# CrystalSixone/VLN-GOAT

Hardware: AMD Instinct MI355X
Metric: trajectory-steps/sec fwd+bwd (GOAT pretrain, 36 views x 768, 80 tok) (higher is better)
Workload: dtype bf16

## Files before the change

include/goat_hip.h:

```cpp
#ifndef GOAT_HIP_H
#define GOAT_HIP_H

#include <stdint.h>

#ifdef __cplusplus
extern "C" {
#endif

#define GOAT_F32 0
#define GOAT_BF16 1

#define GOAT_E_ARG (-1)
#define GOAT_E_SHAPE (-2)

#define GOAT_EPI_NONE 0
#define GOAT_EPI_GELU 1
#define GOAT_EPI_RELU 2
#define GOAT_EPI_MUL_DGELU 3
#define GOAT_EPI_MUL_DRELU 4
#define GOAT_EPI_ACCUM 5

int goat_version(void);

int goat_gemm_nt(void* stream, int dtype_in, int dtype_out,
                 const void* A, int64_t lda, const void* B, int64_t ldb, void* C, int64_t ldc,
                 int M, int N, int K, const float* bias, int epilogue,
                 void* aux, int64_t ldaux, int split_k);

#define GOAT_GEMM_8WAVES 0x100
#define GOAT_GEMM_PP 0x200
#define GOAT_GEMM_PERSIST 0x400

int goat_gemm_bf16(void* stream, int trans_a, int trans_b, int dtype_out,
                   const void* A, int64_t lda, const void* B, int64_t ldb, void* C, int64_t ldc,
                   int M, int N, int Kc, const float* bias, int epilogue,
                   void* aux, int64_t ldaux, int split_k, int bm, int nstage, float* colsum);
int goat_colsum(void* stream, int dtype, const void* x, int64_t ld, int R, int C, float* colsum);

int goat_wgrad_smallk(void* stream, int dtype, const void* dy, int64_t ld_dy, const void* x, int64_t ld_x, int rows, int N, int K,
                      float* dw, int64_t ld_dw, float* dbias);

int goat_transpose(void* stream, int dtype, const void* in, int64_t ld_in, void* out, int64_t ld_out,
                   int R, int C, float* colsum);

int goat_ln_fwd(void* stream, int dtype, const void* x, const void* residual,
                const float* gamma, const float* beta, float eps,
                float p, uint64_t seed, uint64_t offset, const uint64_t* rng_dev,
                void* y, void* z_out, float* mean, float* rstd, int M, int H);

#define GOAT_LN_ADD_BEFORE 4
typedef struct goat_ln_partial {
  const float* ws;
  float* dgamma;
  float* dbeta;
  int32_t nparts;
  int32_t reserved;
} goat_ln_partial;
int goat_ln_bwd_ws_floats(int H);
int goat_ln_bwd_nparts(int M);
// ... 177 lines not shown
```

vln-goat_amd/_lib.py:

```python
import ctypes
import glob
import os
import subprocess

import torch

_HERE = os.path.dirname(os.path.abspath(__file__))
CSRC = os.path.join(_HERE, 'csrc')
LIB_PATH = os.environ.get('GOAT_HIP_LIB') or os.path.join(CSRC, 'libgoat_hip.so')
SOURCES = ['gemm.hip', 'gemm2.hip', 'gemm3.hip', 'gemm5.hip', 'attention.hip', 'attention2.hip', 'attention_long.hip', 'decode.hip', 'rowops.hip', 'causal.hip', 'optim.hip', 'glue.hip']

GOAT_F32, GOAT_BF16 = 0, 1
EPI_NONE, EPI_GELU, EPI_RELU, EPI_MUL_DGELU, EPI_MUL_DRELU, EPI_ACCUM = 0, 1, 2, 3, 4, 5

_lib = None

_vp = ctypes.c_void_p
_i32 = ctypes.c_int
_i64 = ctypes.c_int64
_u64 = ctypes.c_uint64
_f32 = ctypes.c_float

SIGNATURES = {
    'goat_version': [],
    'goat_gemm_nt': [_vp, _i32, _i32, _vp, _i64, _vp, _i64, _vp, _i64, _i32, _i32, _i32, _vp, _i32, _vp, _i64, _i32],
    'goat_gemm_bf16': [_vp, _i32, _i32, _i32, _vp, _i64, _vp, _i64, _vp, _i64, _i32, _i32, _i32, _vp, _i32, _vp, _i64, _i32, _i32, _i32, _vp],
    'goat_colsum': [_vp, _i32, _vp, _i64, _i32, _i32, _vp],
    'goat_transpose': [_vp, _i32, _vp, _i64, _vp, _i64, _i32, _i32, _vp],
    'goat_ln_fwd': [_vp, _i32, _vp, _vp, _vp, _vp, _f32, _f32, _u64, _u64, _vp, _vp, _vp, _vp, _vp, _i32, _i32],
    'goat_wgrad_smallk': [_vp, _i32, _vp, _i64, _vp, _i64, _i32, _i32, _i32, _vp, _i64, _vp],
    'goat_ln_bwd_ws_floats': [_i32],
    'goat_ln_bwd_nparts': [_i32],
    'goat_ln_reduce_batched': [_vp, _vp, _i32, _i32],
    'goat_ln_bwd': [_vp, _i32, _vp, _vp, _vp, _vp, _vp, _vp, _f32, _u64, _u64, _vp, _vp, _vp, _vp, _vp, _vp, _i32, _i32, _i32, _vp],
    'goat_ln_fwd_do': [_vp, _i32, _vp, _vp, _vp, _vp, _f32, _f32, _u64, _u64, _vp, _vp, _vp, _vp, _vp, _i32, _i32, _f32, _u64, _vp],
    'goat_ln_bwd_do': [_vp, _i32, _vp, _vp, _vp, _vp, _vp, _vp, _f32, _u64, _u64, _vp, _vp, _vp, _vp, _vp, _vp, _i32, _i32, _i32, _vp, _f32, _u64, _vp],
    'goat_dropout_add_fwd': [_vp, _i32, _vp, _vp, _vp, _i64, _f32, _u64, _u64, _vp],
    'goat_dropout_bwd': [_vp, _i32, _vp, _vp, _i64, _f32, _u64, _u64, _vp],
    'goat_act_bwd': [_vp, _i32, _vp, _vp, _vp, _i64, _i32, _f32, _u64, _u64, _vp],
    'goat_attn_fwd': [_vp, _i32] + [_vp, _i64, _i64] * 4 + [_vp, _vp, _vp, _i32, _i32, _i32, _i32, _f32, _f32, _u64, _u64, _vp],
    'goat_attn_bwd': [_vp, _i32] + [_vp, _i64, _i64] * 8 + [_vp, _vp, _vp, _vp, _i32, _i32, _i32, _i32, _f32, _f32, _u64, _u64, _vp],
    'goat_attn_long_fwd': [_vp, _i32] + [_vp, _i64, _i64] * 4 + [_vp, _vp, _vp, _i32, _i32, _i32, _i32, _f32, _f32, _u64, _u64, _vp],
    'goat_attn_long_bwd': [_vp, _i32] + [_vp, _i64, _i64] * 8 + [_vp, _vp, _vp, _vp, _i32, _i32, _i32, _i32, _f32, _f32, _u64, _u64, _vp],
    'goat_attn_decode_fwd': [_vp, _i32, _vp, _vp, _vp, _i64, _i64, _vp, _vp, _vp, _i32, _i32, _i32, _f32, _f32, _u64, _u64, _vp],
    'goat_decode_select': [_vp, _vp, _i64, _i32, _i32, _i32, _i32, _i32, _i32, _i32, _u64, _u64, _vp, _vp, _vp, _vp, _vp, _vp, _vp],
    'goat_ce_fwd': [_vp, _vp, _i64, _i32, _i32, _vp, _vp, _vp],
    'goat_ce_bwd': [_vp, _i32, _vp, _i64, _i32, _i32, _vp, _vp, _vp, _vp, _i64],
    'goat_pano_fusion_fwd': [_vp, _i32, _vp, _vp, _vp, _vp, _vp, _i32, _i32, _i32],
    'goat_pano_fusion_bwd': [_vp, _i32, _vp, _vp, _vp, _vp, _vp, _vp, _vp, _vp, _i32, _i32, _i32],
# ... 98 lines not shown
```

vln-goat_amd/csrc/gemm2.hip:

```cpp
#include "gemm5_tile.hpp"

using namespace goat_g2;

static int pick_group_m(int tiles_m, int tiles_n, int bm, int bn) {
  if (const char* e = getenv("GOAT_GEMM_GROUP_M")) {
    int g = atoi(e);
    return g < 1 ? 1 : (g > tiles_m ? tiles_m : g);
  }
  static std::mutex mu;
  static std::unordered_map<uint64_t, int> cache;
  const uint64_t key = ((uint64_t)tiles_m << 44) | ((uint64_t)tiles_n << 24) | ((uint64_t)bm << 12) | (uint64_t)bn;
  {
    std::lock_guard<std::mutex> lk(mu);
    auto it = cache.find(key);
    if (it != cache.end()) return it->second;
  }
  const int nwg = tiles_m * tiles_n, q = nwg >> 3, r = nwg & 7;
  int best = 1;
  double best_cost = 1e300;
  std::vector<char> seen_m(tiles_m), seen_n(tiles_n);
  const int gmax = tiles_m < 64 ? tiles_m : 64;
  for (int gm = 1; gm <= gmax; ++gm) {
    double cost = 0;
    int pos = 0;
// ... 10 lines not shown
        if (!seen_n[tn]) { seen_n[tn] = 1; ++dn; }
      }
      cost += (double)dm * bm + (double)dn * bn;
    }
    if (cost < best_cost - 1e-9) { best_cost = cost; best = gm; }
  }
  std::lock_guard<std::mutex> lk(mu);
  cache[key] = best;
  return best;
}


static bool tile_ok(int bm, int bn, bool eight) {
  if (bn == 128 && bm == 96) return !eight;
  if (bn == 128) return bm == 64 || bm == 128 || bm == 256 ? (!eight || bm == 128) : false;
  if (eight) return false;
  return (bm == 128 && bn == 256) || (bm == 192 && bn == 256) || (bm == 256 && bn == 192) || (bm == 256 && bn == 256) || (bm == 192 && bn == 192);
}

static bool pp_tile_ok(int bm, int bn, int nstage) {
  return nstage == 2 && ((bm == 256 && bn == 256) || (bm == 192 && bn == 256) || (bm == 128 && bn == 256) || (bm == 256 && bn == 128) || (bm == 128 && bn == 128));
}

extern "C" int goat_gemm_bf16(void* stream, int trans_a, int trans_b, int dtype_out,
                              const void* A, int64_t lda, const void* B, int64_t ldb, void* C, int64_t ldc,
                              int M, int N, int Kc, const float* bias, int epilogue,
                              void* aux, int64_t ldaux, int split_k, int bm, int nstage, float* colsum) {
  if (!A || !B || !C) return GOAT_E_ARG;
  const bool eight = (nstage & GOAT_GEMM_8WAVES) != 0;
  const bool pp = (nstage & GOAT_GEMM_PP) != 0;
  const bool persist = (nstage & GOAT_GEMM_PERSIST) != 0;
  nstage &= ~(GOAT_GEMM_8WAVES | GOAT_GEMM_PP | GOAT_GEMM_PERSIST);
  if (nstage < 2 || nstage > 4) return GOAT_E_ARG;
  if (persist && !pp) return GOAT_E_ARG;
  int bn = (bm >> 16) & 0xFFFF;
  bm &= 0xFFFF;
  if (bn == 0) bn = 128;
  if (colsum && !trans_a) return GOAT_E_ARG;
  if (M <= 0 || N <= 0 || Kc <= 0) return GOAT_E_SHAPE;
  if ((lda % 8) || (ldb % 8)) return GOAT_E_SHAPE;
  if ((reinterpret_cast<uintptr_t>(A) & 15) || (reinterpret_cast<uintptr_t>(B) & 15)) return GOAT_E_SHAPE;
  if ((!trans_a || !trans_b) && (Kc % BK)) return GOAT_E_SHAPE;
  if (trans_a && !trans_b) return GOAT_E_ARG;
  if ((epilogue == GOAT_EPI_MUL_DGELU || epilogue == GOAT_EPI_MUL_DRELU) && (!aux || bias)) return GOAT_E_ARG;
  if (epilogue == GOAT_EPI_ACCUM && (dtype_out != GOAT_F32 || bias)) return GOAT_E_ARG;
  if (split_k > 1 && (dtype_out != GOAT_F32 || (epilogue != GOAT_EPI_NONE && epilogue != GOAT_EPI_ACCUM) || bias)) return GOAT_E_ARG;
  if (pp ? (eight || !pp_tile_ok(bm, bn, nstage)) : !tile_ok(bm, bn, eight)) return GOAT_E_ARG;
  const int64_t a_rows = trans_a ? Kc : M, b_rows = trans_b ? Kc : N;
  const int64_t a_bytes = a_rows * lda * 2, b_bytes = b_rows * ldb * 2;
  if (a_bytes >= (1ll << 31) || b_bytes >= (1ll << 31)) return GOAT_E_SHAPE;

  G2Args a;
  a.A = A; a.B = B; a.C = C; a.bias = bias; a.aux = aux;
  a.lda = lda; a.ldb = ldb; a.ldc = ldc; a.ldaux = ldaux;
  a.M = M; a.N = N; a.Kc = Kc;
  a.tiles_m = (M + bm - 1) / bm;
  a.tiles_n = (N + bn - 1) / bn;
  a.a_bytes = (uint32_t)a_bytes; a.b_bytes = (uint32_t)b_bytes;
  a.colsum = colsum;
  a.accum = epilogue == GOAT_EPI_ACCUM;
  a.group_m = pick_group_m(a.tiles_m, a.tiles_n, bm, bn);
  const int kt = (Kc + BK - 1) / BK;
  if (split_k < 1) split_k = 1;
  if (split_k > kt) split_k = kt;
  a.k_tiles_per_split = (kt + split_k - 1) / split_k;
  hipStream_t st = reinterpret_cast<hipStream_t>(stream);
  if (pp) return goat_g5_dispatch(st, a, bm, bn, trans_a, trans_b, dtype_out, epilogue, split_k, nstage, persist);
  if (bn != 128 || bm == 96) return goat_g3_dispatch(st, a, bm, bn, trans_a, trans_b, dtype_out, epilogue, split_k, nstage);
  if (bm == 64) return dispatch_layout<T64>(st, a, trans_a, trans_b, dtype_out, epilogue, split_k, nstage);
  if (bm == 256) return dispatch_layout<T256>(st, a, trans_a, trans_b, dtype_out, epilogue, split_k, nstage);
  if (eight) return dispatch_layout<T128X8>(st, a, trans_a, trans_b, dtype_out, epilogue, split_k, nstage);
  return dispatch_layout<T128>(st, a, trans_a, trans_b, dtype_out, epilogue, split_k, nstage);
}

template <class CF>
static int group_stages(hipStream_t st, const GroupArgs& g, int nstage) {
  constexpr int STAGE = smem_bytes<CF, true, true, 1>();
  if (nstage == 2) return launch_group<CF, 2>(st, g);
  if constexpr (3 * STAGE <= 160 * 1024) {
    if (nstage == 3) return launch_group<CF, 3>(st, g);
  }
  if constexpr (4 * STAGE <= 160 * 1024 && CF::BM * CF::BN <= 128 * 128) {
    if (nstage == 4) return launch_group<CF, 4>(st, g);
  }
  return GOAT_E_ARG;
}

static int build_group(const goat_wgrad_problem* probs, int n, int bm, int bn, GroupArgs& g) {
  g.n = n;
  int tiles = 0;
  for (int i = 0; i < n; ++i) {
    const goat_wgrad_problem& q = probs[i];
    if (!q.dy || !q.x || !q.dw) return GOAT_E_ARG;
    if (q.rows <= 0 || q.n_out <= 0 || q.n_in <= 0) return GOAT_E_SHAPE;
    if ((q.ld_dy % 8) || (q.ld_x % 8)) return GOAT_E_SHAPE;
// ... 58 lines not shown
```

vln-goat_amd/csrc/gemm2_tile.hpp:

```cpp
#pragma once
#include <algorithm>
#include <cstdlib>
#include <mutex>
#include <type_traits>
#include <unordered_map>
#include <vector>
#include "gemm_epilogue.hpp"

namespace goat_g2 {

constexpr int BK = 64;
#ifndef GOAT_GEMM_FRAG_DEPTH
#define GOAT_GEMM_FRAG_DEPTH 2
#endif
#ifndef GOAT_G2_ROTATED
#define GOAT_G2_ROTATED 0
#endif
#ifndef GOAT_G2_SPREAD
#define GOAT_G2_SPREAD 1
#endif
#ifndef GOAT_G2_SETPRIO
#define GOAT_G2_SETPRIO 0
#endif
#ifndef GOAT_G2_NOEPI
// ... 464 lines not shown
template <class F>
int with_epilogue(int epi, F&& f) {
  switch (epi) {
    case GOAT_EPI_NONE: return f(std::integral_constant<int, GOAT_EPI_NONE>());
    case GOAT_EPI_GELU: return f(std::integral_constant<int, GOAT_EPI_GELU>());
    case GOAT_EPI_RELU: return f(std::integral_constant<int, GOAT_EPI_RELU>());
    case GOAT_EPI_MUL_DGELU: return f(std::integral_constant<int, GOAT_EPI_MUL_DGELU>());
    case GOAT_EPI_MUL_DRELU: return f(std::integral_constant<int, GOAT_EPI_MUL_DRELU>());
  }
  return GOAT_E_ARG;
}

template <class CF, bool TA, bool TB>
int dispatch2(hipStream_t st, const G2Args& a, int dtype_out, int epi, int split, int nstage) {
  if (split > 1) return launch2<CF, TA, TB, float, GOAT_EPI_NONE, true>(st, a, split, nstage);
  if (dtype_out == GOAT_F32) {
    if (epi != GOAT_EPI_NONE && epi != GOAT_EPI_ACCUM) return GOAT_E_ARG;
    return launch2<CF, TA, TB, float, GOAT_EPI_NONE, false>(st, a, 1, nstage);
  }
  if constexpr (TA) {
    if (epi != GOAT_EPI_NONE) return GOAT_E_ARG;
    return launch2<CF, TA, TB, bf16_t, GOAT_EPI_NONE, false>(st, a, 1, nstage);
  }
  return with_epilogue(epi, [&](auto e) { return launch2<CF, TA, TB, bf16_t, decltype(e)::value, false>(st, a, 1, nstage); });
}

template <class CF>
int dispatch_layout(hipStream_t st, const G2Args& a, int trans_a, int trans_b, int dtype_out, int epi, int split, int nstage) {
  constexpr bool POW2_M = (CF::BM & (CF::BM - 1)) == 0, POW2_N = (CF::BN & (CF::BN - 1)) == 0;
  if (!trans_a && !trans_b) return dispatch2<CF, false, false>(st, a, dtype_out, epi, split, nstage);
  if constexpr (POW2_N) {
    if (!trans_a && trans_b) return dispatch2<CF, false, true>(st, a, dtype_out, epi, split, nstage);
    if constexpr (POW2_M) {
      if (trans_a && trans_b) return dispatch2<CF, true, true>(st, a, dtype_out, epi, split, nstage);
    }
  }
  return GOAT_E_ARG;
}

template <class CF, int NSTAGE>
int launch_group(hipStream_t st, const GroupArgs& g) {
  constexpr int SMEM = smem_bytes<CF, true, true, NSTAGE>();
  auto kern = gemm2_group_kernel<CF, NSTAGE>;
  static bool attr_set = false;
  if (!attr_set) {
    hipError_t e = hipFuncSetAttribute(reinterpret_cast<const void*>(kern), hipFuncAttributeMaxDynamicSharedMemorySize, SMEM);
// ... 14 lines not shown
```

vln-goat_amd/csrc/gemm5_tile.hpp:

```cpp
#pragma once
#include "gemm2_tile.hpp"
#include "gemm_epilogue.hpp"

namespace goat_g5 {
using namespace goat_g2;

#ifndef GOAT_G5_SETPRIO
#define GOAT_G5_SETPRIO 1
#endif

#ifndef GOAT_G5_TIMING
#define GOAT_G5_TIMING 0
#endif
__device__ __forceinline__ uint32_t g5_now() {
  uint64_t t;
  asm volatile("s_memtime %0\n\ts_waitcnt lgkmcnt(0)" : "=s"(t)::"memory");
  return (uint32_t)t;
}

template <int MI_, int NI_, int NB_, int VAR_ = 0>
struct PCfg {
  static constexpr int MI = MI_, NI = NI_, NB = NB_, VAR = VAR_;
  static constexpr int BM = 64 * MI, BN = 128 * NI, NTH = 512;
  static constexpr int AH = MI * 4096;
// ... 403 lines not shown
      if (do_colsum) {
#pragma unroll
        for (int i = 0; i < MI; ++i)
          bsum[i] += __hip_atomic_load(sk->part_in - (int64_t)c * sk->slot_floats + BS0 + (wave * MI + i) * 64 + lane, __ATOMIC_RELAXED, __HIP_MEMORY_SCOPE_SYSTEM);
      }
      asm volatile("s_waitcnt vmcnt(0)" ::: "memory");
      if (lane == 0) __hip_atomic_store(fl, 0u, __ATOMIC_RELAXED, __HIP_MEMORY_SCOPE_AGENT);
    }
    }
  }
  if (TA && do_colsum) {
#pragma unroll
    for (int i = 0; i < MI; ++i) {
      if (BS_SPLIT && i != wn) continue;
      float v = bsum[i] + __shfl_xor(bsum[i], 32, 64);
      const int row = m0 + wrow0 + i * 32 + l31;
      if (hi == 0 && row < p.M) atomicAdd(p.colsum + row, v);
    }
  }
  if constexpr (SPLITK || sizeof(OutT) == 4) {
    store_tile_f32<MI, NI, SPLITK, true, true>(p, accs, m0 + wrow0, n0 + wcol0, lane);
  } else {
    static_assert(8 * Staging<NI>::WSLICE <= CF::SMEM, "per-wave epilogue slices must fit the LDS ring");
    store_tile_bf16<MI, NI, EPI, 3>(p, accs, smem + wave * Staging<NI>::WSLICE, m0 + wrow0, n0 + wcol0, lane);
  }
#endif
}

template <class CF, bool TA, bool TB, typename OutT, int EPI, bool SPLITK>
__global__ __launch_bounds__(512) void pp_kernel(G2Args p) {
  pp_tile<CF, TA, TB, OutT, EPI, SPLITK>(p, xcd_chunk_position(blockIdx.x, gridDim.x), blockIdx.y);
}

template <class CF>
__global__ __launch_bounds__(512) void pp_group_kernel(GroupArgs g) {
  const int pos = xcd_chunk_position(blockIdx.x, gridDim.x);
  int pi = 0;
#pragma unroll
  for (int i = 1; i < GROUP_MAX; ++i)
    if (i < g.n && pos >= g.tile_start[i]) pi = i;
  const G2Args p = g.prob[pi].template expand<CF::BM, CF::BN>();
  pp_tile<CF, true, true, float, GOAT_EPI_NONE, false>(p, pos - g.tile_start[pi], 0);
}

struct SkGroupArgs {
  GroupArgs g;
  int iter_start[GROUP_MAX + 1];
// ... 72 lines not shown
  static bool attr_set = false;
  if (!attr_set) {
    hipError_t e = hipFuncSetAttribute(reinterpret_cast<const void*>(kern), hipFuncAttributeMaxDynamicSharedMemorySize, CF::SMEM);
    if (e != hipSuccess) return (int)e;
    attr_set = true;
  }
  dim3 grid(a.tiles_m * a.tiles_n, SPLITK ? split : 1);
  hipLaunchKernelGGL(kern, grid, dim3(512), CF::SMEM, st, a);
  GOAT_LAUNCH_CHECK();
  return 0;
}

template <class CF, bool TA, bool TB>
int pp_dispatch2(hipStream_t st, const G2Args& a, int dtype_out, int epi, int split) {
  if (split > 1) return pp_launch<CF, TA, TB, float, GOAT_EPI_NONE, true>(st, a, split);
  if (dtype_out == GOAT_F32) {
    if (epi != GOAT_EPI_NONE && epi != GOAT_EPI_ACCUM) return GOAT_E_ARG;
    return pp_launch<CF, TA, TB, float, GOAT_EPI_NONE, false>(st, a, 1);
  }
  if constexpr (TA) {
    if (epi != GOAT_EPI_NONE) return GOAT_E_ARG;
    return pp_launch<CF, TA, TB, bf16_t, GOAT_EPI_NONE, false>(st, a, 1);
  } else {
    return with_epilogue(epi, [&](auto e) { return pp_launch<CF, TA, TB, bf16_t, decltype(e)::value, false>(st, a, 1); });
  }
}

template <class CF>
int pp_dispatch_layout(hipStream_t st, const G2Args& a, int trans_a, int trans_b, int dtype_out, int epi, int split) {
  if (!trans_a && !trans_b) return pp_dispatch2<CF, false, false>(st, a, dtype_out, epi, split);
  if (!trans_a && trans_b) return pp_dispatch2<CF, false, true>(st, a, dtype_out, epi, split);
  if constexpr ((CF::MI & (CF::MI - 1)) == 0) {
    if (trans_a && trans_b) return pp_dispatch2<CF, true, true>(st, a, dtype_out, epi, split);
  }
  return GOAT_E_ARG;
}

template <class CF>
int pp_launch_group(hipStream_t st, const GroupArgs& g) {
  auto kern = pp_group_kernel<CF>;
  static bool attr_set = false;
  if (!attr_set) {
    hipError_t e = hipFuncSetAttribute(reinterpret_cast<const void*>(kern), hipFuncAttributeMaxDynamicSharedMemorySize, CF::SMEM);
    if (e != hipSuccess) return (int)e;
    attr_set = true;
  }
// ... 262 lines not shown
  }
  return n;
}

template <class CF, bool TB, int EPI>
int pp_launch_persist(hipStream_t st, const G2Args& a) {
  static_assert(CF::SMEM <= 160 * 1024, "LDS exceeds the CU's 160 KiB");
  auto kern = pp_persist_kernel<CF, TB, EPI>;
  static bool attr_set = false;
  if (!attr_set) {
    hipError_t e = hipFuncSetAttribute(reinterpret_cast<const void*>(kern), hipFuncAttributeMaxDynamicSharedMemorySize, CF::SMEM);
    if (e != hipSuccess) return (int)e;
    attr_set = true;
  }
  const int nt = a.tiles_m * a.tiles_n, slots = pp_cu_count() * (CF::SMEM <= 80 * 1024 ? 2 : 1);
  hipLaunchKernelGGL(kern, dim3(nt < slots ? nt : slots), dim3(512), CF::SMEM, st, a);
  GOAT_LAUNCH_CHECK();
  return 0;
}

template <class CF>
int pp_dispatch_persist(hipStream_t st, const G2Args& a, int trans_a, int trans_b, int dtype_out, int epi, int split) {
  if (trans_a || split > 1 || dtype_out != GOAT_BF16) return GOAT_E_ARG;
  if (!trans_b) return with_epilogue(epi, [&](auto e) { return pp_launch_persist<CF, false, decltype(e)::value>(st, a); });
  return with_epilogue(epi, [&](auto e) { return pp_launch_persist<CF, true, decltype(e)::value>(st, a); });
}

}

int goat_g5_dispatch(hipStream_t st, const goat_g2::G2Args& a, int bm, int bn, int trans_a, int trans_b, int dtype_out, int epi,
                     int split, int nstage, bool persist);
int goat_g5_group(hipStream_t st, const goat_g2::GroupArgs& g, int bm, int bn, int nstage);
int goat_g5_group_sk(hipStream_t st, const goat_g2::GroupArgs& g, int bm, int bn, int nstage, void* ws, int64_t ws_bytes);
int64_t goat_g5_group_sk_ws_bytes(int bm, int bn);
```

vln-goat_amd/csrc/gemm_args.hpp:

```cpp
#pragma once
#include "common.hpp"

namespace goat_g2 {

struct G2Args {
  const void* A; const void* B; void* C; const float* bias; void* aux;
  int64_t lda, ldb, ldc, ldaux;
  int M, N, Kc;
  int tiles_m, tiles_n;
  int k_tiles_per_split;
  uint32_t a_bytes, b_bytes;
  float* colsum;
  int accum;
  int group_m;
};

}
```

vln-goat_amd/csrc/gemm_epilogue.hpp:

```cpp
#pragma once
#include "gemm_args.hpp"

namespace goat_g2 {

#ifndef GOAT_G2_STORE
#define GOAT_G2_STORE 1
#endif
typedef uint32_t g2_u32x4 __attribute__((ext_vector_type(4)));
__device__ __forceinline__ void store16(void* dst, const uint4& v) {
#if GOAT_G2_STORE == 1
  const g2_u32x4 q = {v.x, v.y, v.z, v.w};
  asm volatile("global_store_dwordx4 %0, %1, off nt\n\ts_nop 1" ::"v"(dst), "v"(q) : "memory");
#elif GOAT_G2_STORE == 2
  const g2_u32x4 q = {v.x, v.y, v.z, v.w};
  asm volatile("global_store_dwordx4 %0, %1, off sc1\n\ts_nop 1" ::"v"(dst), "v"(q) : "memory");
#else
  *reinterpret_cast<uint4*>(dst) = v;
#endif
}

template <int CHUNKS, int CPR>
__device__ __forceinline__ void load_aux_rows(const G2Args& p, int row_w, int col_w, int lane, uint4* dst) {
  constexpr int EPC = 8;
  const bf16_t* auxp = reinterpret_cast<const bf16_t*>(p.aux);
// ... 35 lines not shown
        if (row < p.M && col < p.N) {
          float* dst = C + (int64_t)row * p.ldc + col;
          const float u = acc[i][j][r] + bcol;
          if (ATOMIC) atomicAdd(dst, acc[i][j][r]);
          else if (p.accum) *dst = u + *dst;
          else if (NT) __builtin_nontemporal_store(u, dst);
          else *dst = u;
        }
      }
    }
}

template <int NI>
struct Staging {
  static constexpr int EPC = 8;
  static constexpr int WCOLS = 32 * NI;
  static constexpr int RBY = WCOLS * 2 + 16;
  static constexpr int WSLICE = 32 * RBY;
  static constexpr int CPR = WCOLS / EPC;
  static constexpr int CHUNKS = 32 * CPR / 64;
  static_assert(32 * CPR % 64 == 0, "a block row is a whole number of 16-byte chunks per lane");
};

constexpr bool epi_is_dact(int epi) { return epi == GOAT_EPI_MUL_DGELU || epi == GOAT_EPI_MUL_DRELU; }
constexpr bool epi_is_act(int epi) { return epi == GOAT_EPI_GELU || epi == GOAT_EPI_RELU; }

template <int NI, int EPI, int AHEAD>
struct AuxAhead {
  static constexpr bool ON = epi_is_dact(EPI) && AHEAD > 0;
  uint4 v[ON ? AHEAD : 1][Staging<NI>::CHUNKS];
};

template <int MI, int NI, int EPI, int AHEAD, int PRIMED>
__device__ __forceinline__ void store_tile_bf16(const G2Args& p, const AccTile<MI, NI> accs, char* wsp, int row0, int col0, int lane,
                                                AuxAhead<NI, EPI, AHEAD>& ahead) {
  const f32x16 (&acc)[MI][NI] = accs.t;
  typedef bf16_t T;
  typedef Staging<NI> S;
  constexpr int EPC = S::EPC, RBY = S::RBY, CPR = S::CPR, CHUNKS = S::CHUNKS;
  constexpr bool DACT = epi_is_dact(EPI), ACT = epi_is_act(EPI);
  constexpr int AD = AHEAD < MI ? AHEAD : MI;
  static_assert(AHEAD >= 0 && AHEAD <= 3 && PRIMED >= 0 && PRIMED <= AD, "prefetch policy: 0..3 block rows ahead, the first PRIMED of them by the caller");
  const int hi = lane >> 5, l31 = lane & 31;
  T* aux = reinterpret_cast<T*>(p.aux);
  T* C = reinterpret_cast<T*>(p.C);
  const bool c_vec = (p.ldc % EPC) == 0 && ((reinterpret_cast<uintptr_t>(C) & 15) == 0);
  const bool aux_vec = aux != nullptr && (p.ldaux % EPC) == 0 && ((reinterpret_cast<uintptr_t>(aux) & 15) == 0);
  f32x4 bv[DACT ? 1 : NI][4];
  if (!DACT) {
#pragma unroll
    for (int j = 0; j < NI; ++j)
#pragma unroll
      for (int q = 0; q < 4; ++q) {
        const int col = col0 + j * 32 + 4 * hi + 8 * q;
#pragma unroll
        for (int e = 0; e < 4; ++e) bv[j][q][e] = (p.bias != nullptr && col + e < p.N) ? p.bias[col + e] : 0.f;
      }
  }
  if constexpr (DACT) {
#pragma unroll
    for (int i = PRIMED; i < AD; ++i) load_aux_rows<CHUNKS, CPR>(p, row0 + i * 32, col0, lane, ahead.v[i]);
  }
#pragma unroll
  for (int i = 0; i < MI; ++i) {
    const int row_w = row0 + i * 32;
    if constexpr (DACT) {
#pragma unroll
      for (int c = 0; c < CHUNKS; ++c) {
        const int idx = c * 64 + lane, r = idx / CPR, cc = idx % CPR;
        uint4 now;
        if constexpr (AD > 0) now = ahead.v[i % AD][c];
        else load_aux_rows<1, CPR>(p, row_w, col0, idx, &now);
        *reinterpret_cast<uint4*>(wsp + r * RBY + cc * 16) = now;
      }
      if constexpr (AD > 0) {
        if (i + AD < MI) load_aux_rows<CHUNKS, CPR>(p, row_w + AD * 32, col0, lane, ahead.v[i % AD]);
      }
      asm volatile("s_waitcnt lgkmcnt(0)" ::: "memory");
    }
#pragma unroll
    for (int j = 0; j < NI; ++j)
#pragma unroll
      for (int q = 0; q < 4; ++q) {
        char* slot = wsp + l31 * RBY + (j * 32 + 4 * hi + 8 * q) * 2;
        float u[4];
#pragma unroll
        for (int e = 0; e < 4; ++e) u[e] = DACT ? acc[i][j][4 * q + e] : acc[i][j][4 * q + e] + bv[DACT ? 0 : j][q][e];
        if (DACT) {
          const bf16x4 a4 = *reinterpret_cast<const bf16x4*>(slot);
#pragma unroll
          for (int e = 0; e < 4; ++e) {
            const float av = (float)a4[e];
            u[e] = (EPI == GOAT_EPI_MUL_DGELU) ? u[e] * dgelu_fast(av) : (av > 0.f ? u[e] : 0.f);
          }
        }
        bf16x4 o4;
#pragma unroll
        for (int e = 0; e < 4; ++e) o4[e] = (bf16_t)u[e];
        *reinterpret_cast<bf16x4*>(slot) = o4;
      }
    asm volatile("s_waitcnt lgkmcnt(0)" ::: "memory");
#pragma unroll
    for (int c = 0; c < CHUNKS; ++c) {
      const int idx = c * 64 + lane, r = idx / CPR, cc = idx % CPR;
      const int row = row_w + r, col = col0 + cc * EPC;
      uint4 raw = *reinterpret_cast<const uint4*>(wsp + r * RBY + cc * 16);
      if (row >= p.M || col >= p.N) continue;
      if (ACT) {
        if (aux != nullptr) {
          if (col + EPC <= p.N && aux_vec) {
            store16(aux + (int64_t)row * p.ldaux + col, raw);
          } else {
            const T* rv = reinterpret_cast<const T*>(&raw);
            for (int e = 0; e < EPC; ++e)
              if (col + e < p.N) aux[(int64_t)row * p.ldaux + col + e] = rv[e];
          }
        }
        bf16x8 v = *reinterpret_cast<bf16x8*>(&raw);
#pragma unroll
        for (int e = 0; e < EPC; ++e) {
          const float u = (float)v[e];
          const float h = (EPI == GOAT_EPI_GELU) ? gelu_fast(u) : fmaxf(u, 0.f);
          v[e] = (bf16_t)h;
        }
        raw = *reinterpret_cast<uint4*>(&v);
      }
      if (col + EPC <= p.N && c_vec) {
        store16(C + (int64_t)row * p.ldc + col, raw);
      } else {
        const T* rv = reinterpret_cast<const T*>(&raw);
        for (int e = 0; e < EPC; ++e)
          if (col + e < p.N) C[(int64_t)row * p.ldc + col + e] = rv[e];
      }
    }
    asm volatile("s_waitcnt lgkmcnt(0)" ::: "memory");
  }
}
template <int MI, int NI, int EPI, int AHEAD>
__device__ __forceinline__ void store_tile_bf16(const G2Args& p, const AccTile<MI, NI> accs, char* wsp, int row0, int col0, int lane) {
  AuxAhead<NI, EPI, AHEAD> ahead;
  store_tile_bf16<MI, NI, EPI, AHEAD, 0>(p, accs, wsp, row0, col0, lane, ahead);
}

}
```

vln-goat_amd/csrc/rowops.hip:

```cpp
#include <cstdlib>
#include "common.hpp"
#include <algorithm>
#include <vector>

namespace {

#ifndef GOAT_LN_ABL
#define GOAT_LN_ABL 0
#endif
constexpr int MAXC_MAX = 8;

template <typename T, int MAXC>
__global__ __launch_bounds__(256) void ln_fwd_kernel(const T* __restrict__ x, const T* __restrict__ res,
                                                     const float* __restrict__ gamma, const float* __restrict__ beta,
                                                     float eps, float p, uint64_t seed, uint64_t offset,
                                                     const uint64_t* __restrict__ rng_dev, T* __restrict__ y, T* __restrict__ zout, float* __restrict__ mean,
                                                     float* __restrict__ rstd, int M, int H, float p_out, uint64_t offset_out,
                                                     const T* __restrict__ post_add) {
  constexpr int EPC = DT<T>::EPC;
  const int lane = threadIdx.x & 63;
  const int row = blockIdx.x * 4 + (threadIdx.x >> 6);
  if (row >= M) return;
  if (rng_dev) seed += *rng_dev;
  const GoatRng rng(seed);
// ... 1137 lines not shown
template <typename T>
int ln_check(int H) {
  const int epc = DT<T>::EPC;
  if (H % epc) return GOAT_E_SHAPE;
  if (H > 64 * MAXC_MAX * epc) return GOAT_E_SHAPE;
  return 0;
}
template <typename T>
int ln_maxc(int H) {
  const int need = (H / DT<T>::EPC + 63) / 64;
  return need <= 1 ? 1 : need <= 2 ? 2 : need <= 3 ? 3 : need <= 4 ? 4 : 8;
}
#define GOAT_LN_DISPATCH(T_, H_, ...)                        \
  switch (ln_maxc<T_>(H_)) {                                 \
    case 1: { constexpr int MC = 1; __VA_ARGS__; } break;    \
    case 2: { constexpr int MC = 2; __VA_ARGS__; } break;    \
    case 3: { constexpr int MC = 3; __VA_ARGS__; } break;    \
    case 4: { constexpr int MC = 4; __VA_ARGS__; } break;    \
    default: { constexpr int MC = 8; __VA_ARGS__; } break;   \
  }

}

extern "C" int goat_version(void) { return 103; }

extern "C" int goat_ln_fwd_do(void* stream, int dtype, const void* x, const void* residual, const float* gamma,
                              const float* beta, float eps, float p, uint64_t seed, uint64_t offset,
                              const uint64_t* rng_dev, void* y, void* z_out, float* mean, float* rstd, int M, int H, float p_out,
                              uint64_t offset_out, const void* post_add) {
  if (!x || !gamma || !beta || !y || !mean || !rstd) return GOAT_E_ARG;
  if (M <= 0 || !(p_out >= 0.f && p_out < 1.f)) return GOAT_E_SHAPE;
  if ((residual || p > 0.f) && !z_out) return GOAT_E_ARG;
  dim3 grid((M + 3) / 4);
  return dtype_dispatch(dtype, [&](auto dt) -> int {
    typedef GOAT_DT_TYPE(dt) T;
    if (int e = ln_check<T>(H)) return e;
    GOAT_LN_DISPATCH(T, H, hipLaunchKernelGGL((ln_fwd_kernel<T, MC>), grid, dim3(256), 0, ST(stream), (const T*)x, (const T*)residual, gamma,
                                              beta, eps, p, seed, offset, rng_dev, (T*)y, (T*)z_out, mean, rstd, M, H, p_out, offset_out,
                                              (const T*)post_add));
    GOAT_LAUNCH_CHECK();
    return 0;
  });
}

extern "C" int goat_ln_fwd(void* stream, int dtype, const void* x, const void* residual, const float* gamma,
                           const float* beta, float eps, float p, uint64_t seed, uint64_t offset,
                           const uint64_t* rng_dev, void* y, void* z_out, float* mean, float* rstd, int M, int H) {
// ... 401 lines not shown
```

vln-goat_amd/hipops.py:

```python
import ctypes
import json
import math
import os

import torch

from . import _lib
from ._lib import GOAT_BF16, GOAT_F32, EPI_ACCUM, EPI_GELU, EPI_MUL_DGELU, EPI_MUL_DRELU, EPI_NONE, EPI_RELU

_ACT_EPI = {None: EPI_NONE, 'none': EPI_NONE, 'gelu': EPI_GELU, 'relu': EPI_RELU}
_ACT_DEPI = {'gelu': EPI_MUL_DGELU, 'relu': EPI_MUL_DRELU}


from ._plumbing import _dt, _epc, _need_gpu, _ptr, _stream


class RngState:
    seed = None
    rank_salt = 0
    base = None
    counter = 0
    dev = None

    @classmethod
# ... 336 lines not shown
        return (dx.view(ctx.xshape) if dx is not None else None), dw, db


ROWDOT = os.environ.get('GOAT_NO_ROWDOT', '0') != '1'


def linear(x, weight, bias=None, act=None, out_dtype=None):
    if (ROWDOT and weight.shape[0] == 1 and act in (None, 'none') and out_dtype is None and x.is_cuda and x.shape[-1] == weight.shape[1]
            and weight.shape[1] % 8 == 0 and weight.shape[1] <= 1024 and weight.dtype == torch.float32 and weight.is_contiguous()
            and (bias is None or bias.dtype == torch.float32) and x.dtype in (torch.float32, torch.bfloat16)):
        return _RowDotFn.apply(x, weight, bias)
    return _LinearFn.apply(x, weight, bias, act, out_dtype)


def act_bwd(dy, u, act, p=0.0, rng=(0, 0, None)):
    dy = dy if dy.is_contiguous() else dy.contiguous()
    dx = torch.empty_like(dy)
    st = _lib.lib().goat_act_bwd(_stream(), _dt(dy), _ptr(dy), _ptr(u), _ptr(dx), dy.numel(), _ACT_EPI[act],
                                 p, rng[0], rng[1], rng[2])
    _lib.check(st, 'goat_act_bwd')
    return dx


class _FfnFn(torch.autograd.Function):

    @staticmethod
    def forward(ctx, x, w1, b1, w2, b2, act, p):
        _need_gpu(x)
        x2 = _rows(x)
        W1 = _shadow(w1, x2.dtype)
        W2 = _shadow(w2, x2.dtype)
        M, F_ = x2.shape[0], W1.shape[0]
        u = torch.empty((M, F_), dtype=x2.dtype, device=x2.device)
        h = torch.empty_like(u)
        rng = RngState.next(h.numel()) if p > 0 else (0, 0, None)
        gemm(x2, W1, h, bias=b1.detach(), epi=_ACT_EPI[act], aux=u)
        if p > 0:
            st = _lib.lib().goat_dropout_add_fwd(_stream(), _dt(h), _ptr(h), None, _ptr(h), h.numel(), p,
                                                 rng[0], rng[1], rng[2])
            _lib.check(st, 'goat_dropout_add_fwd')
        y = torch.empty((M, W2.shape[0]), dtype=x2.dtype, device=x2.device)
        gemm(h, W2, y, bias=b2.detach())
        ctx.save_for_backward(x2, u, h)
        ctx.w1, ctx.w2, ctx.act, ctx.xshape, ctx.p, ctx.rng = w1, w2, act, x.shape, p, rng
        ctx.b1, ctx.b2 = b1, b2
        return y.view(*x.shape[:-1], W2.shape[0])

    @staticmethod
    def backward(ctx, dy):
        x2, u, h = ctx.saved_tensors
        dy2 = _rows(dy)
        W2 = _shadow(ctx.w2, x2.dtype)
        du = torch.empty_like(u)
        if ctx.p > 0:
            gemm(dy2, W2, du, tb=True)
            du = act_bwd(du, u, ctx.act, ctx.p, ctx.rng)
        else:
            gemm(dy2, W2, du, tb=True, epi=_ACT_DEPI[ctx.act], aux=u)
        dw2, db2 = linear_wgrad(dy2, h, (ctx.w2,), (ctx.b2,))
        W1 = _shadow(ctx.w1, x2.dtype)
        dx = torch.empty_like(x2)
        gemm(du, W1, dx, tb=True)
        dw1, db1 = linear_wgrad(du, x2, (ctx.w1,), (ctx.b1,))
        return dx.view(ctx.xshape), dw1, db1, dw2, db2, None, None


def ffn(x, w1, b1, w2, b2, act='gelu', p=0.0):
    return _FfnFn.apply(x, w1, b1, w2, b2, act, float(p))


class _DecoderCeFn(torch.autograd.Function):

    @staticmethod
    def forward(ctx, h, weight, bias, targets):
        _need_gpu(h)
        h2 = _rows(h)
        M, K = h2.shape
        N = weight.shape[0]
        Np = (N + 63) // 64 * 64
# ... 1142 lines not shown
```

Baseline: 46530.

## Fuse FFN dropout into GEMM GELU epilogues for forward and backward

Adds GELU+dropout and dGELU+dropout GEMM epilogues that generate keep masks from the counter-based RNG inside the store tile. In backward, the keep bits are staged in padding bytes of the LDS slice. The FFN forward no longer runs a separate dropout pass over h, and the backward no longer runs a separate act_bwd pass over du. This saves a full read-modify-write of the intermediate activation in each direction, at the cost of extra RNG work in the epilogue and a reduced aux prefetch depth for MI=4 tiles.

Result: no change. 46260 (-0.6%).

```diff
diff --git a/include/goat_hip.h b/include/goat_hip.h
--- a/include/goat_hip.h
+++ b/include/goat_hip.h
@@ -35,6 +35,13 @@
                    const void* A, int64_t lda, const void* B, int64_t ldb, void* C, int64_t ldc,
                    int M, int N, int Kc, const float* bias, int epilogue,
                    void* aux, int64_t ldaux, int split_k, int bm, int nstage, float* colsum);
+#define GOAT_EPI_GELU_DROP 6
+#define GOAT_EPI_MUL_DGELU_DROP 7
+int goat_gemm_bf16_ffn_drop(void* stream, int trans_b, int dtype_out,
+                            const void* A, int64_t lda, const void* B, int64_t ldb, void* C, int64_t ldc,
+                            int M, int N, int Kc, const float* bias, int epilogue,
+                            void* aux, int64_t ldaux, int split_k, int bm, int nstage,
+                            float p, uint64_t seed, uint64_t offset, const uint64_t* rng_dev);
 int goat_colsum(void* stream, int dtype, const void* x, int64_t ld, int R, int C, float* colsum);
 
 int goat_wgrad_smallk(void* stream, int dtype, const void* dy, int64_t ld_dy, const void* x, int64_t ld_x, int rows, int N, int K,
diff --git a/vln-goat_amd/_lib.py b/vln-goat_amd/_lib.py
--- a/vln-goat_amd/_lib.py
+++ b/vln-goat_amd/_lib.py
@@ -12,6 +12,7 @@
 
 GOAT_F32, GOAT_BF16 = 0, 1
 EPI_NONE, EPI_GELU, EPI_RELU, EPI_MUL_DGELU, EPI_MUL_DRELU, EPI_ACCUM = 0, 1, 2, 3, 4, 5
+EPI_GELU_DROP, EPI_MUL_DGELU_DROP = 6, 7
 
 _lib = None
 
@@ -25,6 +26,7 @@
     'goat_version': [],
     'goat_gemm_nt': [_vp, _i32, _i32, _vp, _i64, _vp, _i64, _vp, _i64, _i32, _i32, _i32, _vp, _i32, _vp, _i64, _i32],
     'goat_gemm_bf16': [_vp, _i32, _i32, _i32, _vp, _i64, _vp, _i64, _vp, _i64, _i32, _i32, _i32, _vp, _i32, _vp, _i64, _i32, _i32, _i32, _vp],
+    'goat_gemm_bf16_ffn_drop': [_vp, _i32, _i32, _vp, _i64, _vp, _i64, _vp, _i64, _i32, _i32, _i32, _vp, _i32, _vp, _i64, _i32, _i32, _i32, _f32, _u64, _u64, _vp],
     'goat_colsum': [_vp, _i32, _vp, _i64, _i32, _i32, _vp],
     'goat_transpose': [_vp, _i32, _vp, _i64, _vp, _i64, _i32, _i32, _vp],
     'goat_ln_fwd': [_vp, _i32, _vp, _vp, _vp, _vp, _f32, _f32, _u64, _u64, _vp, _vp, _vp, _vp, _vp, _i32, _i32],
diff --git a/vln-goat_amd/csrc/gemm2.hip b/vln-goat_amd/csrc/gemm2.hip
--- a/vln-goat_amd/csrc/gemm2.hip
+++ b/vln-goat_amd/csrc/gemm2.hip
@@ -56,11 +56,14 @@
   return nstage == 2 && ((bm == 256 && bn == 256) || (bm == 192 && bn == 256) || (bm == 128 && bn == 256) || (bm == 256 && bn == 128) || (bm == 128 && bn == 128));
 }
 
-extern "C" int goat_gemm_bf16(void* stream, int trans_a, int trans_b, int dtype_out,
-                              const void* A, int64_t lda, const void* B, int64_t ldb, void* C, int64_t ldc,
-                              int M, int N, int Kc, const float* bias, int epilogue,
-                              void* aux, int64_t ldaux, int split_k, int bm, int nstage, float* colsum) {
+struct DropArgs { float p; uint64_t seed, offset; const uint64_t* rng_dev; };
+
+static int gemm_bf16(void* stream, int trans_a, int trans_b, int dtype_out,
+                     const void* A, int64_t lda, const void* B, int64_t ldb, void* C, int64_t ldc,
+                     int M, int N, int Kc, const float* bias, int epilogue,
+                     void* aux, int64_t ldaux, int split_k, int bm, int nstage, float* colsum, const DropArgs* drop) {
   if (!A || !B || !C) return GOAT_E_ARG;
+  if (!drop && (epilogue == GOAT_EPI_GELU_DROP || epilogue == GOAT_EPI_MUL_DGELU_DROP)) return GOAT_E_ARG;
   const bool eight = (nstage & GOAT_GEMM_8WAVES) != 0;
   const bool pp = (nstage & GOAT_GEMM_PP) != 0;
   const bool persist = (nstage & GOAT_GEMM_PERSIST) != 0;
@@ -76,7 +79,7 @@
   if ((reinterpret_cast<uintptr_t>(A) & 15) || (reinterpret_cast<uintptr_t>(B) & 15)) return GOAT_E_SHAPE;
   if ((!trans_a || !trans_b) && (Kc % BK)) return GOAT_E_SHAPE;
   if (trans_a && !trans_b) return GOAT_E_ARG;
-  if ((epilogue == GOAT_EPI_MUL_DGELU || epilogue == GOAT_EPI_MUL_DRELU) && (!aux || bias)) return GOAT_E_ARG;
+  if ((epilogue == GOAT_EPI_MUL_DGELU || epilogue == GOAT_EPI_MUL_DRELU || epilogue == GOAT_EPI_MUL_DGELU_DROP) && (!aux || bias)) return GOAT_E_ARG;
   if (epilogue == GOAT_EPI_ACCUM && (dtype_out != GOAT_F32 || bias)) return GOAT_E_ARG;
   if (split_k > 1 && (dtype_out != GOAT_F32 || (epilogue != GOAT_EPI_NONE && epilogue != GOAT_EPI_ACCUM) || bias)) return GOAT_E_ARG;
   if (pp ? (eight || !pp_tile_ok(bm, bn, nstage)) : !tile_ok(bm, bn, eight)) return GOAT_E_ARG;
@@ -94,6 +97,10 @@
   a.colsum = colsum;
   a.accum = epilogue == GOAT_EPI_ACCUM;
   a.group_m = pick_group_m(a.tiles_m, a.tiles_n, bm, bn);
+  a.drop_p = drop ? drop->p : 0.f;
+  a.drop_seed = drop ? drop->seed : 0;
+  a.drop_offset = drop ? drop->offset : 0;
+  a.drop_rng_dev = drop ? drop->rng_dev : nullptr;
   const int kt = (Kc + BK - 1) / BK;
   if (split_k < 1) split_k = 1;
   if (split_k > kt) split_k = kt;
@@ -105,6 +112,35 @@
   if (bm == 256) return dispatch_layout<T256>(st, a, trans_a, trans_b, dtype_out, epilogue, split_k, nstage);
   if (eight) return dispatch_layout<T128X8>(st, a, trans_a, trans_b, dtype_out, epilogue, split_k, nstage);
   return dispatch_layout<T128>(st, a, trans_a, trans_b, dtype_out, epilogue, split_k, nstage);
+}
+
+extern "C" int goat_gemm_bf16(void* stream, int trans_a, int trans_b, int dtype_out,
+                              const void* A, int64_t lda, const void* B, int64_t ldb, void* C, int64_t ldc,
+                              int M, int N, int Kc, const float* bias, int epilogue,
+                              void* aux, int64_t ldaux, int split_k, int bm, int nstage, float* colsum) {
+  return gemm_bf16(stream, trans_a, trans_b, dtype_out, A, lda, B, ldb, C, ldc, M, N, Kc, bias, epilogue, aux, ldaux, split_k, bm, nstage,
+                   colsum, nullptr);
+}
+
+extern "C" int goat_gemm_bf16_ffn_drop(void* stream, int trans_b, int dtype_out,
+                                       const void* A, int64_t lda, const void* B, int64_t ldb, void* C, int64_t ldc,
+                                       int M, int N, int Kc, const float* bias, int epilogue,
+                                       void* aux, int64_t ldaux, int split_k, int bm, int nstage,
+                                       float p, uint64_t seed, uint64_t offset, const uint64_t* rng_dev) {
+  if (!A || !B || !C || !aux) return GOAT_E_ARG;
+  const bool fwd = epilogue == GOAT_EPI_GELU_DROP, bwd = epilogue == GOAT_EPI_MUL_DGELU_DROP;
+  if (!fwd && !bwd) return GOAT_E_ARG;
+  if (fwd ? trans_b != 0 : (trans_b == 0 || bias != nullptr)) return GOAT_E_ARG;
+  if (dtype_out != GOAT_BF16 || split_k > 1) return GOAT_E_ARG;
+  if (!(p >= 0.f && p < 1.f)) return GOAT_E_ARG;
+  if (N <= 0 || (N % 8) || ldc != N || ldaux != N || (offset % 8)) return GOAT_E_ARG;
+  if ((reinterpret_cast<uintptr_t>(C) & 15) || (reinterpret_cast<uintptr_t>(aux) & 15)) return GOAT_E_ARG;
+  if (M > 0 && (int64_t)M * N >= (1ll << 40)) return GOAT_E_ARG;
+  if (p == 0.f)
+    return gemm_bf16(stream, 0, trans_b, dtype_out, A, lda, B, ldb, C, ldc, M, N, Kc, bias, fwd ? GOAT_EPI_GELU : GOAT_EPI_MUL_DGELU, aux,
+                     ldaux, 1, bm, nstage, nullptr, nullptr);
+  const DropArgs drop = {p, seed, offset, rng_dev};
+  return gemm_bf16(stream, 0, trans_b, dtype_out, A, lda, B, ldb, C, ldc, M, N, Kc, bias, epilogue, aux, ldaux, 1, bm, nstage, nullptr, &drop);
 }
 
 template <class CF>
diff --git a/vln-goat_amd/csrc/gemm2_tile.hpp b/vln-goat_amd/csrc/gemm2_tile.hpp
--- a/vln-goat_amd/csrc/gemm2_tile.hpp
+++ b/vln-goat_amd/csrc/gemm2_tile.hpp
@@ -510,6 +510,10 @@
     if (epi != GOAT_EPI_NONE) return GOAT_E_ARG;
     return launch2<CF, TA, TB, bf16_t, GOAT_EPI_NONE, false>(st, a, 1, nstage);
   }
+  if (epi == GOAT_EPI_GELU_DROP || epi == GOAT_EPI_MUL_DGELU_DROP) {
+    constexpr int DROP_EPI = TB ? GOAT_EPI_MUL_DGELU_DROP : GOAT_EPI_GELU_DROP;
+    return epi == DROP_EPI ? launch2<CF, TA, TB, bf16_t, DROP_EPI, false>(st, a, 1, nstage) : GOAT_E_ARG;
+  }
   return with_epilogue(epi, [&](auto e) { return launch2<CF, TA, TB, bf16_t, decltype(e)::value, false>(st, a, 1, nstage); });
 }
 
diff --git a/vln-goat_amd/csrc/gemm5_tile.hpp b/vln-goat_amd/csrc/gemm5_tile.hpp
--- a/vln-goat_amd/csrc/gemm5_tile.hpp
+++ b/vln-goat_amd/csrc/gemm5_tile.hpp
@@ -449,7 +449,7 @@
     store_tile_f32<MI, NI, SPLITK, true, true>(p, accs, m0 + wrow0, n0 + wcol0, lane);
   } else {
     static_assert(8 * Staging<NI>::WSLICE <= CF::SMEM, "per-wave epilogue slices must fit the LDS ring");
-    store_tile_bf16<MI, NI, EPI, 3>(p, accs, smem + wave * Staging<NI>::WSLICE, m0 + wrow0, n0 + wcol0, lane);
+    store_tile_bf16<MI, NI, EPI, (MI == 4 && epi_is_drop(EPI) ? 2 : 3)>(p, accs, smem + wave * Staging<NI>::WSLICE, m0 + wrow0, n0 + wcol0, lane);
   }
 #endif
 }
@@ -568,6 +568,10 @@
     if (epi != GOAT_EPI_NONE) return GOAT_E_ARG;
     return pp_launch<CF, TA, TB, bf16_t, GOAT_EPI_NONE, false>(st, a, 1);
   } else {
+    if (epi == GOAT_EPI_GELU_DROP || epi == GOAT_EPI_MUL_DGELU_DROP) {
+      constexpr int DROP_EPI = TB ? GOAT_EPI_MUL_DGELU_DROP : GOAT_EPI_GELU_DROP;
+      return epi == DROP_EPI ? pp_launch<CF, TA, TB, bf16_t, DROP_EPI, false>(st, a, 1) : GOAT_E_ARG;
+    }
     return with_epilogue(epi, [&](auto e) { return pp_launch<CF, TA, TB, bf16_t, decltype(e)::value, false>(st, a, 1); });
   }
 }
@@ -876,6 +880,11 @@
 template <class CF>
 int pp_dispatch_persist(hipStream_t st, const G2Args& a, int trans_a, int trans_b, int dtype_out, int epi, int split) {
   if (trans_a || split > 1 || dtype_out != GOAT_BF16) return GOAT_E_ARG;
+  if (epi == GOAT_EPI_GELU_DROP) return trans_b ? GOAT_E_ARG : pp_launch_persist<CF, false, GOAT_EPI_GELU_DROP>(st, a);
+  if (epi == GOAT_EPI_MUL_DGELU_DROP) {
+    if constexpr (CF::BM == 256 && CF::BN == 256) return GOAT_E_ARG;
+    else return trans_b ? pp_launch_persist<CF, true, GOAT_EPI_MUL_DGELU_DROP>(st, a) : GOAT_E_ARG;
+  }
   if (!trans_b) return with_epilogue(epi, [&](auto e) { return pp_launch_persist<CF, false, decltype(e)::value>(st, a); });
   return with_epilogue(epi, [&](auto e) { return pp_launch_persist<CF, true, decltype(e)::value>(st, a); });
 }
diff --git a/vln-goat_amd/csrc/gemm_args.hpp b/vln-goat_amd/csrc/gemm_args.hpp
--- a/vln-goat_amd/csrc/gemm_args.hpp
+++ b/vln-goat_amd/csrc/gemm_args.hpp
@@ -13,6 +13,9 @@
   float* colsum;
   int accum;
   int group_m;
+  float drop_p;
+  uint64_t drop_seed, drop_offset;
+  const uint64_t* drop_rng_dev;
 };
 
 }
diff --git a/vln-goat_amd/csrc/gemm_epilogue.hpp b/vln-goat_amd/csrc/gemm_epilogue.hpp
--- a/vln-goat_amd/csrc/gemm_epilogue.hpp
+++ b/vln-goat_amd/csrc/gemm_epilogue.hpp
@@ -81,8 +81,9 @@
   static_assert(32 * CPR % 64 == 0, "a block row is a whole number of 16-byte chunks per lane");
 };
 
-constexpr bool epi_is_dact(int epi) { return epi == GOAT_EPI_MUL_DGELU || epi == GOAT_EPI_MUL_DRELU; }
-constexpr bool epi_is_act(int epi) { return epi == GOAT_EPI_GELU || epi == GOAT_EPI_RELU; }
+constexpr bool epi_is_dact(int epi) { return epi == GOAT_EPI_MUL_DGELU || epi == GOAT_EPI_MUL_DRELU || epi == GOAT_EPI_MUL_DGELU_DROP; }
+constexpr bool epi_is_act(int epi) { return epi == GOAT_EPI_GELU || epi == GOAT_EPI_RELU || epi == GOAT_EPI_GELU_DROP; }
+constexpr bool epi_is_drop(int epi) { return epi == GOAT_EPI_GELU_DROP || epi == GOAT_EPI_MUL_DGELU_DROP; }
 
 template <int NI, int EPI, int AHEAD>
 struct AuxAhead {
@@ -97,7 +98,8 @@
   typedef bf16_t T;
   typedef Staging<NI> S;
   constexpr int EPC = S::EPC, RBY = S::RBY, CPR = S::CPR, CHUNKS = S::CHUNKS;
-  constexpr bool DACT = epi_is_dact(EPI), ACT = epi_is_act(EPI);
+  constexpr bool DACT = epi_is_dact(EPI), ACT = epi_is_act(EPI), DROP = epi_is_drop(EPI);
+  static_assert(!DROP || CPR <= 16, "one keep byte per chunk in the 16 padding bytes of a slice row");
   constexpr int AD = AHEAD < MI ? AHEAD : MI;
   static_assert(AHEAD >= 0 && AHEAD <= 3 && PRIMED >= 0 && PRIMED <= AD, "prefetch policy: 0..3 block rows ahead, the first PRIMED of them by the caller");
   const int hi = lane >> 5, l31 = lane & 31;
@@ -116,6 +118,9 @@
         for (int e = 0; e < 4; ++e) bv[j][q][e] = (p.bias != nullptr && col + e < p.N) ? p.bias[col + e] : 0.f;
       }
   }
+  const GoatRng rng(DROP ? p.drop_seed + (p.drop_rng_dev ? *p.drop_rng_dev : 0ull) : 0ull);
+  const uint32_t thr = DROP ? goat_thr16(p.drop_p) : 0u;
+  const float ks = DROP ? 1.f / (1.f - p.drop_p) : 1.f;
   if constexpr (DACT) {
 #pragma unroll
     for (int i = PRIMED; i < AD; ++i) load_aux_rows<CHUNKS, CPR>(p, row0 + i * 32, col0, lane, ahead.v[i]);
@@ -131,11 +136,20 @@
         if constexpr (AD > 0) now = ahead.v[i % AD][c];
         else load_aux_rows<1, CPR>(p, row_w, col0, idx, &now);
         *reinterpret_cast<uint4*>(wsp + r * RBY + cc * 16) = now;
+        if constexpr (DROP) {
+          const uint64_t ctr = (p.drop_offset + (uint64_t)((int64_t)(row_w + r) * p.N + (col0 + cc * EPC))) & ~(uint64_t)7;
+          *reinterpret_cast<uint8_t*>(wsp + r * RBY + S::WCOLS * 2 + cc) = (uint8_t)rng.keep_bits<EPC>(ctr, thr);
+        }
       }
       if constexpr (AD > 0) {
         if (i + AD < MI) load_aux_rows<CHUNKS, CPR>(p, row_w + AD * 32, col0, lane, ahead.v[i % AD]);
       }
       asm volatile("s_waitcnt lgkmcnt(0)" ::: "memory");
+    }
+    uint32_t keepw[DROP && DACT ? NI : 1];
+    if constexpr (DROP && DACT) {
+#pragma unroll
+      for (int j = 0; j < NI; ++j) keepw[j] = *reinterpret_cast<const uint32_t*>(wsp + l31 * RBY + S::WCOLS * 2 + j * 4);
     }
 #pragma unroll
     for (int j = 0; j < NI; ++j)
@@ -147,10 +161,18 @@
         for (int e = 0; e < 4; ++e) u[e] = DACT ? acc[i][j][4 * q + e] : acc[i][j][4 * q + e] + bv[DACT ? 0 : j][q][e];
         if (DACT) {
           const bf16x4 a4 = *reinterpret_cast<const bf16x4*>(slot);
+          uint32_t km = 0;
+          if constexpr (DROP) km = keepw[j] >> (8 * q + 4 * hi);
 #pragma unroll
           for (int e = 0; e < 4; ++e) {
             const float av = (float)a4[e];
-            u[e] = (EPI == GOAT_EPI_MUL_DGELU) ? u[e] * dgelu_fast(av) : (av > 0.f ? u[e] : 0.f);
+            if constexpr (DROP) {
+              float g = (float)(bf16_t)u[e];
+              g = ((km >> e) & 1u) ? g * ks : 0.f;
+              u[e] = g * dgelu_f(av);
+            } else {
+              u[e] = (EPI == GOAT_EPI_MUL_DGELU) ? u[e] * dgelu_fast(av) : (av > 0.f ? u[e] : 0.f);
+            }
           }
         }
         bf16x4 o4;
@@ -176,11 +198,14 @@
           }
         }
         bf16x8 v = *reinterpret_cast<bf16x8*>(&raw);
+        uint32_t km = 0;
+        if constexpr (DROP) km = rng.keep_bits<EPC>((p.drop_offset + (uint64_t)((int64_t)row * p.N + col)) & ~(uint64_t)7, thr);
 #pragma unroll
         for (int e = 0; e < EPC; ++e) {
           const float u = (float)v[e];
-          const float h = (EPI == GOAT_EPI_GELU) ? gelu_fast(u) : fmaxf(u, 0.f);
+          const float h = (EPI == GOAT_EPI_GELU || EPI == GOAT_EPI_GELU_DROP) ? gelu_fast(u) : fmaxf(u, 0.f);
           v[e] = (bf16_t)h;
+          if constexpr (DROP) v[e] = (bf16_t)(((km >> e) & 1u) ? (float)v[e] * ks : 0.f);
         }
         raw = *reinterpret_cast<uint4*>(&v);
       }
diff --git a/vln-goat_amd/csrc/rowops.hip b/vln-goat_amd/csrc/rowops.hip
--- a/vln-goat_amd/csrc/rowops.hip
+++ b/vln-goat_amd/csrc/rowops.hip
@@ -1183,7 +1183,7 @@
 
 }
 
-extern "C" int goat_version(void) { return 103; }
+extern "C" int goat_version(void) { return 104; }
 
 extern "C" int goat_ln_fwd_do(void* stream, int dtype, const void* x, const void* residual, const float* gamma,
                               const float* beta, float eps, float p, uint64_t seed, uint64_t offset,
diff --git a/vln-goat_amd/hipops.py b/vln-goat_amd/hipops.py
--- a/vln-goat_amd/hipops.py
+++ b/vln-goat_amd/hipops.py
@@ -382,6 +382,56 @@
     return dx
 
 
+FFN_DROP_FUSE = os.environ.get('GOAT_NO_FFN_DROP_FUSE', '0') != '1'
+
+
+def _ffn_drop_cfg(tb, M, N, Kc, a, b, out, bias, aux):
+    keys = [(False, tb, M, N, Kc, EPI_MUL_DGELU if tb else EPI_GELU, False, 1, bias is not None)]
+    if tb:
+        keys.append((False, True, M, N, Kc, EPI_NONE, False, 1, False))
+    for key in keys:
+        cfg = _TUNED.get(key)
+        if cfg is not None:
+            tuning.STATS['gemm_tuned'] += 1
+            bm, ns = cfg[:2]
+            if tb and bm == tile(256, 256) and ns & PERSIST:
+                ns &= ~PERSIST
+            return bm, ns
+    key = keys[-1]
+    if tuning.AUTOTUNE and not torch.cuda.is_current_stream_capturing() and tuning.PROFILE is None:
+        return _tune_gemm(key, a, b, out, False, tb, M, N, Kc, bias, key[5], aux if key[5] != EPI_NONE else None, (1,), None)[:2]
+    tuning.STATS['gemm_heuristic'] += 1
+    if len(tuning.STATS_LOG) < 256:
+        tuning.STATS_LOG.append(('gemm', key, bool(torch.cuda.is_current_stream_capturing())))
+    return _heuristic_cfg(False, tb, M, N, Kc, 1)
+
+
+def gemm_ffn_drop(a, b, out, tb, bias, aux, p, rng, cfg=None):
+    M, Kc = a.shape
+    N = b.shape[1] if tb else b.shape[0]
+    assert (b.shape[0] if tb else b.shape[1]) == Kc and out.shape == (M, N) and aux.shape == (M, N)
+    if not (a.dtype == torch.bfloat16 and out.dtype == torch.bfloat16 and M > 0 and N % 8 == 0 and Kc > 0 and (tb or Kc % 64 == 0)
+            and a.stride(1) == 1 and b.stride(1) == 1 and a.stride(0) % 8 == 0 and b.stride(0) % 8 == 0
+            and a.data_ptr() % 16 == 0 and b.data_ptr() % 16 == 0 and out.is_contiguous() and aux.is_contiguous()
+            and out.data_ptr() % 16 == 0 and aux.data_ptr() % 16 == 0 and rng[1] % 8 == 0):
+        return False
+    bm, nstage = cfg if cfg is not None else _ffn_drop_cfg(tb, M, N, Kc, a, b, out, bias, aux)
+    epi = _lib.EPI_MUL_DGELU_DROP if tb else _lib.EPI_GELU_DROP
+    cargs = (int(tb), _dt(out), _ptr(a), a.stride(0), _ptr(b), b.stride(0), _ptr(out), out.stride(0), M, N, Kc,
+             _ptr(bias) if bias is not None else None, epi, _ptr(aux), aux.stride(0), 1, bm, nstage, p, rng[0], rng[1], rng[2])
+    ev = _profile_start() if tuning.PROFILE is not None else None
+    st = _lib.lib().goat_gemm_bf16_ffn_drop(_stream(), *cargs)
+    if st == -1:
+        return False
+    _lib.check(st, 'goat_gemm_bf16_ffn_drop(tb=%d,M=%d,N=%d,Kc=%d,bm=%d,ns=%d)' % (tb, M, N, Kc, bm, nstage))
+    if ev is not None:
+        ev[1].record()
+        tuning.PROFILE.append(ev + (2.0 * M * N * Kc, (M, N, Kc, EPI_MUL_DGELU if tb else EPI_GELU, 1,
+                                                     'v2 t0%d %s %s drop' % (tb, tile_name(bm), stage_name(nstage))),
+                                    ('goat_gemm_bf16_ffn_drop', cargs, (a, b, out, bias, aux))))
+    return True
+
+
 class _FfnFn(torch.autograd.Function):
 
     @staticmethod
@@ -394,11 +444,12 @@
         u = torch.empty((M, F_), dtype=x2.dtype, device=x2.device)
         h = torch.empty_like(u)
         rng = RngState.next(h.numel()) if p > 0 else (0, 0, None)
-        gemm(x2, W1, h, bias=b1.detach(), epi=_ACT_EPI[act], aux=u)
-        if p > 0:
-            st = _lib.lib().goat_dropout_add_fwd(_stream(), _dt(h), _ptr(h), None, _ptr(h), h.numel(), p,
-                                                 rng[0], rng[1], rng[2])
-            _lib.check(st, 'goat_dropout_add_fwd')
+        if not (p > 0 and FFN_DROP_FUSE and act == 'gelu' and gemm_ffn_drop(x2, W1, h, False, b1.detach(), u, p, rng)):
+            gemm(x2, W1, h, bias=b1.detach(), epi=_ACT_EPI[act], aux=u)
+            if p > 0:
+                st = _lib.lib().goat_dropout_add_fwd(_stream(), _dt(h), _ptr(h), None, _ptr(h), h.numel(), p,
+                                                     rng[0], rng[1], rng[2])
+                _lib.check(st, 'goat_dropout_add_fwd')
         y = torch.empty((M, W2.shape[0]), dtype=x2.dtype, device=x2.device)
         gemm(h, W2, y, bias=b2.detach())
         ctx.save_for_backward(x2, u, h)
@@ -413,8 +464,9 @@
         W2 = _shadow(ctx.w2, x2.dtype)
         du = torch.empty_like(u)
         if ctx.p > 0:
-            gemm(dy2, W2, du, tb=True)
-            du = act_bwd(du, u, ctx.act, ctx.p, ctx.rng)
+            if not (FFN_DROP_FUSE and ctx.act == 'gelu' and gemm_ffn_drop(dy2, W2, du, True, None, u, ctx.p, ctx.rng)):
+                gemm(dy2, W2, du, tb=True)
+                du = act_bwd(du, u, ctx.act, ctx.p, ctx.rng)
         else:
             gemm(dy2, W2, du, tb=True, epi=_ACT_DEPI[ctx.act], aux=u)
         dw2, db2 = linear_wgrad(dy2, h, (ctx.w2,), (ctx.b2,))
```
